# codihuston/eioku

Hardware: AMD Instinct MI355X
Metric: frames/sec (scene+detect+embed) per node (higher is better)
Workload: dtype f16

## Files before the change

### eioku_amd/csrc/yolo.hip

```cpp
#include <algorithm>
#include <array>
#include <memory>
#include <string>
#include <vector>

#include "convnet.h"
#include "yolo_ops.h"

#include <cstdlib>

using namespace eioku;

namespace {

constexpr int kRegMax = 16;

struct Buf {
  int level;
  int ch;
  DevBuf<__half> ptr;
};

enum OpKind { kConv, kPool, kUp };

struct Op {
  OpKind kind;
  int conv = -1;
  int in_buf, in_off, in_ch;
  int out_buf, out_off;
  int res_buf = -1, res_off = 0;
  int act = kActSiLU;
  int f32_out = -1;
  bool pose = false;
  bool chain_next = false;
  bool sole_consumer = false;
  int up_consumer = -1;
  int up_from = -1;
};

}

struct eioku_yolo {
  int ch[5], depth[4], nc, nk = 0;
  ConvStack convs;
  std::vector<Buf> bufs;
  std::vector<Op> ops;
  int in_buf = -1;
  int head_src[3];
  int cur_n = 0, cur_h = 0, cur_w = 0;
  DevBuf<float> head[9];
  DevBuf<float> kpts;
  DevBuf<unsigned long long> clsmax[3];
  DevBuf<int32_t> lvl;
  DevBuf<int32_t> flat;
  int32_t* pass_host = nullptr;
  hipEvent_t pass_event = nullptr;
  bool pass_pending = false;
  long long pass_seen[2] = {0, 0};
  int deep_idx[3][2] = {{-1, -1}, {-1, -1}, {-1, -1}};
  DevBuf<Cand> cands;
  DevBuf<int32_t> counts;
  DevBuf<Det> dets;
  DevBuf<char> lb_tables;
  unsigned long long lb_key = 0;
  void* lb_key_ptr = nullptr;
  __half* lb_out = nullptr;
  double conv_flops_last = 0;
};

namespace {

int add_buf(eioku_yolo* y, int level, int ch) {
  y->bufs.push_back(Buf{level, ch, {}});
  return (int)y->bufs.size() - 1;
}

int add_conv_w(eioku_yolo* y, const std::string& name, int cout, int cin, int k, int s) {
  return y->convs.add({name, cout, cin, k, s});
}

void add_conv(eioku_yolo* y, const std::string& name, int cin, int cout, int k, int s, int in_buf, int in_off,
              int out_buf, int out_off, int res_buf = -1, int res_off = 0, int act = kActSiLU, int f32_out = -1) {
  Op op;
  op.kind = kConv;
  op.conv = add_conv_w(y, name, cout, cin, k, s);
  op.in_buf = in_buf;
  op.in_off = in_off;
  op.in_ch = cin;
  op.out_buf = out_buf;
  op.out_off = out_off;
  op.res_buf = res_buf;
  op.res_off = res_off;
  op.act = act;
  op.f32_out = f32_out;
  y->ops.push_back(op);
}

void add_c2f(eioku_yolo* y, const std::string& p, int level, int c1, int c2, int n, bool shortcut, int in_buf,
             int in_off, int out_buf, int out_off) {
  const int c = c2 / 2;
  const int cat = add_buf(y, level, (2 + n) * c);
  const int tmp = add_buf(y, level, c);
  add_conv(y, p + ".cv1.conv", c1, 2 * c, 1, 1, in_buf, in_off, cat, 0);
  for (int i = 0; i < n; ++i) {
    const std::string m = p + ".m." + std::to_string(i);
    add_conv(y, m + ".cv1.conv", c, c, 3, 1, cat, (1 + i) * c, tmp, 0);
    add_conv(y, m + ".cv2.conv", c, c, 3, 1, tmp, 0, cat, (2 + i) * c, shortcut ? cat : -1, (1 + i) * c);
  }
// ... 110 lines not shown
    if (c.kind == kConv && y->convs.layers[c.conv].k == 1 && c.in_off == 0 && c.in_ch >= up.in_ch && up.in_ch % 32 == 0) {
      up.up_consumer = consumer;
      c.up_from = (int)i;
    }
  }
  for (size_t i = 0; i + 1 < y->ops.size(); ++i) {
    Op& op = y->ops[i];
    if (op.kind != kConv || op.f32_out >= 0 || op.out_buf == y->in_buf) continue;
    int readers = 0;
    for (size_t j = 0; j < y->ops.size(); ++j)
      readers += (y->ops[j].in_buf == op.out_buf) + (y->ops[j].res_buf == op.out_buf);
    const Op& nx = y->ops[i + 1];
    int writers = 0;
    for (const Op& o : y->ops) writers += (o.f32_out < 0 && o.out_buf == op.out_buf);
    op.sole_consumer = readers == 1 && writers == 1 && nx.in_buf == op.out_buf && nx.res_buf != op.out_buf &&
                       y->bufs[op.out_buf].ch == y->convs.layers[op.conv].cout;
    bool priv = nx.in_buf == op.out_buf && nx.in_off == op.out_off && y->bufs[op.out_buf].ch == y->convs.layers[op.conv].cout;
    for (size_t j = 0; j < y->ops.size() && priv; ++j) {
      const Op& o = y->ops[j];
      if (o.res_buf == op.out_buf) priv = false;
      if (o.in_buf == op.out_buf) {
        const Op* pv = j > 0 ? &y->ops[j - 1] : nullptr;
        priv = priv && pv && pv->kind == kConv && pv->f32_out < 0 && pv->out_buf == op.out_buf && pv->out_off == o.in_off;
      }
    }
    op.chain_next = priv;
  }
}

int level_dim(int x, int level) {
  for (int i = 0; i < level; ++i) x = conv_out_dim(x, 3, 2);
  return x;
}

int prepare(eioku_yolo* y, int n, int h, int w) {
  EIOKU_REQUIRE(h % 32 == 0 && w % 32 == 0, "network input %dx%d must be a multiple of 32", h, w);
  for (const auto& b : y->bufs) {
    const long long px = (long long)n * level_dim(h, b.level) * level_dim(w, b.level);
    EIOKU_REQUIRE(px * b.ch < (1ll << 31) && px < (1ll << 24) * 16,
                  "batch of %d frames at %dx%d: an activation tensor of %lld x %d channels exceeds one launch's 32-bit "
                  "offsets -- split the batch", n, h, w, px, b.ch);
  }
  for (auto& b : y->bufs) EIOKU_TRY(grow_synced(b.ptr, (size_t)n * level_dim(h, b.level) * level_dim(w, b.level) * b.ch));
  size_t A = 0;
  for (int l = 0; l < 3; ++l) {
    const size_t px = (size_t)n * level_dim(h, 3 + l) * level_dim(w, 3 + l);
    A += px;
    EIOKU_TRY(grow_synced(y->head[l], px * 4 * kRegMax));
    EIOKU_TRY(grow_synced(y->head[3 + l], px * y->nc));
    EIOKU_TRY(grow_synced(y->clsmax[l], px));
    if (y->nk > 0) EIOKU_TRY(grow_synced(y->head[6 + l], px * y->nk));
  }
  EIOKU_TRY(grow_synced(y->cands, A + (A + 3) / 4));
  EIOKU_TRY(grow_synced(y->counts, (size_t)n * 2));
  EIOKU_TRY(grow_synced(y->lvl, A + (size_t)n * 3));
  EIOKU_TRY(grow_synced(y->flat, 10 * A + 16));
  y->cur_n = n;
  y->cur_h = h;
  y->cur_w = w;
  return EIOKU_OK;
}

__global__ void k_pass_record(const int32_t* counts, int n, int total, int32_t* out) {
  __shared__ int s;
  if (threadIdx.x == 0) s = 0;
  __syncthreads();
  int v = 0;
  for (int i = threadIdx.x; i < n; i += blockDim.x) v += counts[i];
  atomicAdd(&s, v);
  __syncthreads();
  if (threadIdx.x == 0) {
    out[0] = s;
    out[1] = 0;
    out[2] = 0;
    out[3] = total;
  }
}

int record_pass_rate(eioku_yolo* y, int n, int A, hipStream_t stream) {
  int32_t* dev = y->flat + (size_t)10 * n * A + 8;
  hipLaunchKernelGGL(k_pass_record, dim3(1), dim3(256), 0, stream, y->counts.p, n, n * A, dev);
  EIOKU_HIP_CHECK(hipMemcpyAsync(y->pass_host, dev, 4 * sizeof(int32_t), hipMemcpyDeviceToHost, stream));
  EIOKU_HIP_CHECK(hipEventRecord(y->pass_event, stream));
  y->pass_pending = true;
  return EIOKU_OK;
}

int run_ops(eioku_yolo* y, int n, int h, int w, hipStream_t stream, const FusedInput* fused, double* flops_out,
            bool clsmax = false, bool lazybox = false, bool lazydeep = false, bool kpts = false) {
  static const bool up_off = env_off("EIOKU_UP_FUSE");
  double flops = 0;
  bool skip_next = false;
  int pool_skip = 0, front_skip = 0;
  for (const Op& op : y->ops) {
    if (front_skip > 0) {
      --front_skip;
      continue;
    }
    if (skip_next) {
      skip_next = false;
      continue;
    }
    if (op.pose && !kpts) continue;
    const Buf& ib = y->bufs[op.in_buf];
    const int H = level_dim(h, ib.level), W = level_dim(w, ib.level);
    Slice in{ib.ptr, ib.ch, op.in_off};
    int rc = EIOKU_OK;
// ... 299 lines not shown
      EIOKU_HIP_CHECK(hipMemcpyAsync((void*)p.xalpha, xalpha, (size_t)p.new_w * 4, hipMemcpyHostToDevice, stream));
      EIOKU_HIP_CHECK(hipMemcpyAsync((void*)p.ybeta, ybeta, (size_t)p.new_h * 4, hipMemcpyHostToDevice, stream));
      EIOKU_HIP_CHECK(hipStreamSynchronize(stream));
      y->lb_key = key;
      y->lb_key_ptr = t;
    }
  }
  const uint8_t* d_bgr = bgr;
  if (mem == EIOKU_MEM_HOST) {
    uint8_t* s = (uint8_t*)scratch(kSlotIn, (size_t)n * h * w * 3);
    if (!s) return EIOKU_ENOMEM;
    EIOKU_HIP_CHECK(hipMemcpyAsync(s, bgr, (size_t)n * h * w * 3, hipMemcpyHostToDevice, stream));
    d_bgr = s;
  }
  int step = 1, off = 0;
  if (p.mode == 1 && p.new_w > 1 && p.new_h > 1) {
    const int k = xofs[1] - xofs[0];
    bool decim = k >= 2 && yofs[1] - yofs[0] == k && xofs[0] == yofs[0] && xofs[0] >= 0 &&
                 (long long)k * (p.new_w - 1) + xofs[0] <= w - 2 && (long long)k * (p.new_h - 1) + yofs[0] < h;
    for (int i = 0; decim && i < p.new_w; ++i) decim = xofs[i] == k * i + xofs[0] && xalpha[2 * i] == 2048 && xalpha[2 * i + 1] == 0;
    for (int j = 0; decim && j < p.new_h; ++j) decim = yofs[j] == k * j + yofs[0] && ybeta[2 * j] == 2048 && ybeta[2 * j + 1] == 0;
    if (decim) {
      step = k;
      off = xofs[0];
    }
  }
  FusedInput fi{d_bgr, p.src_h, p.src_w, p.new_h, p.new_w, p.top, p.left, step > 1 ? 0 : p.mode, step, off};
  const Op& op0 = y->ops.front();
  static const bool no_fuse = env_off("EIOKU_STEM_FUSE");
  const bool fuse = !no_fuse && op0.kind == kConv && op0.in_buf == y->in_buf && op0.res_buf < 0 && op0.f32_out < 0 &&
                    fused_input_ok(y->convs.w[op0.conv], fi, Slice{}, nullptr);
  if (!fuse) {
    rc = letterbox_forward(d_bgr, n, p, y->bufs[y->in_buf].ptr, stream);
    if (rc) return rc;
  }
  bool cm = true;
  for (const Op& op : y->ops)
    if (op.kind == kConv && op.f32_out >= 3 && op.f32_out < 6) cm = cm && conv_clsmax_ok(y->convs.w[op.conv], op.act);
  static const bool lazy_off = env_off("EIOKU_LAZY_BOX");
  bool lazy = cm && !lazy_off;
  LazyBox lbx{};
  for (const Op& op : y->ops)
    if (op.kind == kConv && op.f32_out >= 0 && op.f32_out < 3) {
      const ConvWeights& cw = y->convs.w[op.conv];
      lazy = lazy && cw.ks == 1 && cw.ntiles == 1 && cw.nf == 4 && cw.cout == 64 && cw.cin % 32 == 0 && op.act == kActNone &&
             op.res_buf < 0 && (lbx.in_cs == 0 || (lbx.in_cs == y->bufs[op.in_buf].ch && lbx.nchunks == cw.nchunks));
      lbx.in[op.f32_out] = y->bufs[op.in_buf].ptr + op.in_off;
      lbx.wgt[op.f32_out] = reinterpret_cast<const uint4*>(cw.d_w.p);
      lbx.bias[op.f32_out] = cw.d_b;
      lbx.in_cs = y->bufs[op.in_buf].ch;
      lbx.nchunks = cw.nchunks;
    }
  static const float deep_frac = (float)env_num("EIOKU_LAZY_DEEP_FRAC", 0.03);
  bool deep = lazy && deep_frac > 0.f;
  int Hq[3], Wq[3], Aq = 0;
  for (int l = 0; l < 3; ++l) {
    Hq[l] = level_dim(p.out_h, 3 + l);
    Wq[l] = level_dim(p.out_w, 3 + l);
    Aq += Hq[l] * Wq[l];
  }
  if (deep) {
    if (!y->pass_host) {
      EIOKU_HIP_CHECK(hipHostMalloc((void**)&y->pass_host, 4 * sizeof(int32_t), hipHostMallocDefault));
      EIOKU_HIP_CHECK(hipEventCreateWithFlags(&y->pass_event, hipEventDisableTiming));
      y->pass_host[0] = y->pass_host[1] = y->pass_host[2] = y->pass_host[3] = 0;
    }
    if (y->pass_pending && hipEventQuery(y->pass_event) == hipSuccess) {
      y->pass_seen[0] = (long long)y->pass_host[0] + y->pass_host[1] + y->pass_host[2];
      y->pass_seen[1] = y->pass_host[3];
      y->pass_pending = false;
    }
    const long long passed = y->pass_seen[0], total = y->pass_seen[1];
    deep = total > 0 && (float)passed <= deep_frac * (float)total;
    int32_t* f = y->flat;
    int32_t* fcnt = f + (size_t)10 * n * Aq;
    size_t off1 = 0, off0 = (size_t)n * Aq;
    for (int l = 0; l < 3 && deep; ++l) {
      const int i0 = y->deep_idx[l][0], i1 = y->deep_idx[l][1];
      if (i0 < 0 || i1 < 0) {
        deep = false;
        break;
      }
      const Op& o0 = y->ops[i0];
      const Op& o1 = y->ops[i1];
      const ConvWeights& w0 = y->convs.w[o0.conv];
      const ConvWeights& w1 = y->convs.w[o1.conv];
      auto ok3 = [](const ConvWeights& w, const Op& o) {
        return w.ks == 3 && w.stride == 1 && w.cout == 64 && w.cin % 32 == 0 && o.act == kActSiLU && o.res_buf < 0 && o.f32_out < 0;
      };
      if (!ok3(w0, o0) || !ok3(w1, o1) || (long long)n * Hq[l] * Wq[l] >= (1ll << 31)) {
        deep = false;
        break;
      }
      lbx.c0[l] = LazyConv3{y->bufs[o0.in_buf].ptr + o0.in_off, y->bufs[o0.in_buf].ch, w0.nchunks,
                            reinterpret_cast<const uint4*>(w0.d_w.p), 16 * w0.nf, w0.d_b,
                            y->bufs[o0.out_buf].ptr + o0.out_off, y->bufs[o0.out_buf].ch};
      lbx.c1[l] = LazyConv3{y->bufs[o1.in_buf].ptr + o1.in_off, y->bufs[o1.in_buf].ch, w1.nchunks,
                            reinterpret_cast<const uint4*>(w1.d_w.p), 16 * w1.nf, w1.d_b,
                            y->bufs[o1.out_buf].ptr + o1.out_off, y->bufs[o1.out_buf].ch};
      lbx.flat1[l] = f + off1;
      lbx.flat0[l] = f + off0;
      off1 += (size_t)n * Hq[l] * Wq[l];
      off0 += (size_t)9 * n * Hq[l] * Wq[l];
    }
    lbx.fcnt = fcnt;
    lbx.deep = deep;
  }
  rc = run_network(y, n, p.out_h, p.out_w, stream, fuse ? &fi : nullptr, cm, lazy, deep, kpts_out != nullptr);
  if (rc) return rc;

  int Hl[3], Wl[3], A = 0;
  for (int l = 0; l < 3; ++l) {
    Hl[l] = level_dim(p.out_h, 3 + l);
    Wl[l] = level_dim(p.out_w, 3 + l);
    A += Hl[l] * Wl[l];
  }
  rc = grow_synced(y->dets, (size_t)n * max_det);
  if (rc) return rc;
  EIOKU_HIP_CHECK(hipMemsetAsync(y->counts, 0, (size_t)n * 2 * sizeof(int32_t), stream));
  const float* box[3] = {y->head[0], y->head[1], y->head[2]};
  const float* cls[3] = {y->head[3], y->head[4], y->head[5]};
  const unsigned long long* cmw[3] = {y->clsmax[0], y->clsmax[1], y->clsmax[2]};
  if (lazy) {
    int32_t* lvl_counts = y->lvl + (size_t)n * A;
    EIOKU_HIP_CHECK(hipMemsetAsync(lvl_counts, 0, (size_t)n * 3 * sizeof(int32_t), stream));
    if (lbx.deep) EIOKU_HIP_CHECK(hipMemsetAsync(lbx.fcnt, 0, 6 * sizeof(int32_t), stream));
    float* boxw[3] = {y->head[0], y->head[1], y->head[2]};
    rc = decode_lazy_forward(boxw, cmw, lbx, n, Hl, Wl, y->nc, conf, y->cands, y->counts, y->lvl, lvl_counts, A, stream);
    if (rc == EIOKU_OK && y->pass_host) rc = record_pass_rate(y, n, A, stream);
  } else {
    rc = decode_forward(box, cm ? nullptr : cls, n, Hl, Wl, y->nc, conf, y->cands, y->counts, A, stream, cm ? cmw : nullptr);
  }
  if (rc) return rc;
  ScaleParams sp;
  sp.gain = gain;
  sp.pad_x = (float)lb_geom[7];
  sp.pad_y = (float)lb_geom[8];
  sp.src_w = (float)w;
  sp.src_h = (float)h;
  rc = nms_forward(y->cands, y->counts, n, A, iou, max_det, 7680.0f, sp, y->dets, y->counts + n, stream);
  if (rc) return rc;
  const hipMemcpyKind kind = mem == EIOKU_MEM_HOST ? hipMemcpyDeviceToHost : hipMemcpyDeviceToDevice;
  if (kpts_out) {
    const float* kp[3] = {y->head[6], y->head[7], y->head[8]};
    const ScaleParams kps{gain, (float)(((double)p.out_w - (double)w * (double)gain) / 2), (float)(((double)p.out_h - (double)h * (double)gain) / 2),
                          (float)w, (float)h};
    EIOKU_TRY(grow_synced(y->kpts, (size_t)n * max_det * y->nk));
    rc = kpts_decode_forward(kp, y->dets, y->counts + n, n, Hl, Wl, y->nk, max_det, kps, y->kpts, stream);
    if (rc) return rc;
    EIOKU_HIP_CHECK(hipMemcpyAsync(kpts_out, y->kpts, (size_t)n * max_det * y->nk * sizeof(float), kind, stream));
  }
  EIOKU_HIP_CHECK(hipMemcpyAsync(dets_out, y->dets, (size_t)n * max_det * sizeof(Det), kind, stream));
  EIOKU_HIP_CHECK(hipMemcpyAsync(counts_out, y->counts + n, (size_t)n * sizeof(int32_t), kind, stream));
  if (mem == EIOKU_MEM_HOST) EIOKU_HIP_CHECK(hipStreamSynchronize(stream));
  return EIOKU_OK;
}

}

extern "C" {

int eioku_letterbox_f16(const uint8_t* bgr_dev, int n, int h, int w, const int32_t* lb_geom, const int32_t* xofs,
                        const int32_t* yofs, const int16_t* xalpha, const int16_t* ybeta, void* out_nhwc8_dev,
                        void* stream_) {
  EIOKU_REQUIRE_INIT();
  EIOKU_REQUIRE(lb_geom && (n == 0 || (bgr_dev && out_nhwc8_dev)), "NULL argument");
  hipStream_t stream = (hipStream_t)stream_;
  LetterboxPlan p;
  p.src_h = h; p.src_w = w;
  p.new_h = lb_geom[0]; p.new_w = lb_geom[1]; p.top = lb_geom[2]; p.left = lb_geom[3];
  p.out_h = lb_geom[4]; p.out_w = lb_geom[5]; p.mode = lb_geom[6];
  EIOKU_REQUIRE(p.mode >= 0 && p.mode <= 2, "bad letterbox mode %d", p.mode);
  EIOKU_REQUIRE(p.mode != 1 || (xofs && yofs && xalpha && ybeta), "bilinear letterbox needs its tables");
  char* t = (char*)scratch(kSlotWork0, (size_t)(p.new_w + p.new_h) * 8 + 64);
  if (!t) return EIOKU_ENOMEM;
  p.xofs = (const int32_t*)t;
  p.yofs = (const int32_t*)(t + (size_t)p.new_w * 4);
  p.xalpha = (const int16_t*)(t + (size_t)p.new_w * 4 + (size_t)p.new_h * 4);
  p.ybeta = (const int16_t*)(t + (size_t)p.new_w * 8 + (size_t)p.new_h * 4);
  if (p.mode == 1) {
    for (int i = 0; i < p.new_w; ++i) EIOKU_REQUIRE(xofs[i] >= 0 && xofs[i] < w, "xofs[%d]=%d outside the frame", i, xofs[i]);
    EIOKU_HIP_CHECK(hipMemcpyAsync((void*)p.xofs, xofs, (size_t)p.new_w * 4, hipMemcpyHostToDevice, stream));
    EIOKU_HIP_CHECK(hipMemcpyAsync((void*)p.yofs, yofs, (size_t)p.new_h * 4, hipMemcpyHostToDevice, stream));
    EIOKU_HIP_CHECK(hipMemcpyAsync((void*)p.xalpha, xalpha, (size_t)p.new_w * 4, hipMemcpyHostToDevice, stream));
    EIOKU_HIP_CHECK(hipMemcpyAsync((void*)p.ybeta, ybeta, (size_t)p.new_h * 4, hipMemcpyHostToDevice, stream));
  }
  return letterbox_forward(bgr_dev, n, p, (__half*)out_nhwc8_dev, stream);
}

int eioku_yolo_postprocess(const float* const* box_dev, const float* const* cls_dev, int n, const int* hl,
                           const int* wl, int nc, float conf, float iou, int max_det, float gain, int pad_x,
                           int pad_y, int src_w, int src_h, void* dets_dev, int32_t* counts_dev, void* stream_) {
  return eioku_yolo_postprocess_pose(box_dev, cls_dev, nullptr, n, hl, wl, nc, 0, conf, iou, max_det, gain, pad_x, pad_y, 0.f,
                                     0.f, src_w, src_h, dets_dev, counts_dev, nullptr, stream_);
}

int eioku_yolo_postprocess_pose(const float* const* box_dev, const float* const* cls_dev, const float* const* kpt_dev, int n,
                                const int* hl, const int* wl, int nc, int nk, float conf, float iou, int max_det, float gain,
                                int pad_x, int pad_y, float kpad_x, float kpad_y, int src_w, int src_h, void* dets_dev,
                                int32_t* counts_dev, float* kpts_dev, void* stream_) {
  EIOKU_REQUIRE_INIT();
  EIOKU_REQUIRE(!kpts_dev || (kpt_dev && nk > 0 && nk % 3 == 0), "keypoint output without keypoint maps");
  EIOKU_REQUIRE(box_dev && cls_dev && hl && wl && dets_dev && counts_dev, "NULL argument");
  hipStream_t stream = (hipStream_t)stream_;
  if (n == 0) return EIOKU_OK;
  int A = 0;
// ... 19 lines not shown
```

### eioku_amd/csrc/yolo_ops.h

```cpp
#pragma once

#include "conv.h"

namespace eioku {

struct Det {
  float x1, y1, x2, y2;
  float conf;
  int32_t cls;
  int32_t anchor;
  int32_t pad;
};
static_assert(sizeof(Det) == 32, "Det layout is part of the C ABI");

struct Cand {
  float x1, y1, x2, y2;
  float conf;
  int32_t cls;
  int32_t anchor;
  int32_t pad;
};

struct LetterboxPlan {
  int src_h, src_w;
  int new_h, new_w;
  int top, left;
  int out_h, out_w;
  int mode;
  const int32_t* xofs;
  const int32_t* yofs;
  const int16_t* xalpha;
  const int16_t* ybeta;
};
int letterbox_forward(const uint8_t* bgr, int n, const LetterboxPlan& p, __half* out_nhwc8, hipStream_t stream);

int maxpool5_forward(Slice in, Slice out, int N, int H, int W, int C, hipStream_t stream);
int sppf_pools_forward(Slice in, Slice out, int out_step, int N, int H, int W, int C, hipStream_t stream);
int upsample2x_forward(Slice in, Slice out, int N, int H, int W, int C, hipStream_t stream);

int decode_forward(const float* const box[3], const float* const cls[3], int N, const int Hl[3],
                   const int Wl[3], int nc, float conf_thres, Cand* cands, int32_t* counts,
                   int max_cand, hipStream_t stream, const unsigned long long* const clsmax[3] = nullptr);

struct LazyConv3 {
  const __half* in;
  int in_cs, nchunks;
  const uint4* wgt;
  int rows_tile;
  const float* bias;
  __half* out;
  int out_cs;
};
struct LazyBox {
  const __half* in[3];
  const uint4* wgt[3];
  const float* bias[3];
  int in_cs, nchunks;
  bool deep = false;
  LazyConv3 c0[3], c1[3];
  int32_t* flat1[3];
  int32_t* flat0[3];
  int32_t* fcnt;
};
int decode_lazy_forward(float* const box[3], const unsigned long long* const clsmax[3], const LazyBox& lb, int N,
                        const int Hl[3], const int Wl[3], int nc, float conf_thres, Cand* cands, int32_t* counts,
                        int32_t* lvl_list, int32_t* lvl_counts, int max_cand, hipStream_t stream);

struct ScaleParams {
  float gain;
  float pad_x, pad_y;
  float src_w, src_h;
};
int nms_forward(const Cand* cands, const int32_t* counts, int N, int max_cand, float iou_thres,
                int max_det, float max_wh, ScaleParams sp, Det* dets, int32_t* det_counts,
                hipStream_t stream);

int kpts_decode_forward(const float* const kpt[3], const Det* dets, const int32_t* det_counts, int N, const int Hl[3],
                        const int Wl[3], int nk, int max_det, ScaleParams sp, float* out, hipStream_t stream);

}
```

### eioku_amd/csrc/yolo_ops.hip

```cpp
#include "yolo_ops.h"

namespace eioku {

namespace {

struct LbArgs {
  const uint8_t* bgr;
  __half* out;
  int n, src_h, src_w, new_h, new_w, top, left, out_h, out_w, mode;
  const int32_t* xofs;
  const int32_t* yofs;
  const int16_t* xalpha;
  const int16_t* ybeta;
};

__global__ __launch_bounds__(256) void k_letterbox(LbArgs a) {
  const long long total = (long long)a.n * a.out_h * a.out_w;
  long long i = blockIdx.x * 256ll + threadIdx.x;
  if (i >= total) return;
  const int ox = (int)(i % a.out_w);
  const long long t = i / a.out_w;
  const int oy = (int)(t % a.out_h);
  const int n = (int)(t / a.out_h);
  const int y = oy - a.top, x = ox - a.left;
// ... 279 lines not shown
  bool pass = false;
  if (valid) {
    const unsigned long long word = a.cm[lvl][pix];
    const float best = __uint_as_float((unsigned)(word & 0xFFFFFFFFull));
    conf = 1.0f / (1.0f + expf(-best));
    pass = conf > a.conf;
  }
  if (pass) {
    const int pos = atomicAdd(&a.counts[n], 1);
    a.keys[(size_t)n * a.A + pos] =
        ((unsigned long long)__float_as_uint(conf) << 32) | (unsigned long long)(0xFFFFFFFFu - (unsigned)an);
    const int k = atomicAdd(&a.lvl_counts[n * 3 + lvl], 1);
    a.lvl_list[(size_t)n * a.A + a.A0[lvl] + k] = loc;
  }
  if (!a.fcnt) return;
  const int lane = threadIdx.x & 63;
  const int y = loc / W, x = loc - y * W;
  int nb[9], c = 0;
  if (pass) {
#pragma unroll
    for (int dy = -1; dy <= 1; ++dy)
#pragma unroll
      for (int dx = -1; dx <= 1; ++dx)
        if ((unsigned)(y + dy) < (unsigned)H && (unsigned)(x + dx) < (unsigned)W) nb[c++] = (int)pix + dy * W + dx;
  }
  int incl = c;
#pragma unroll
  for (int off = 1; off < 64; off <<= 1) {
    const int v = __shfl_up(incl, off, 64);
    if (lane >= off) incl += v;
  }
  for (int l = 0; l < 3; ++l) {
    const unsigned long long m = __ballot(pass && lvl == l);
    if (m == 0) continue;
    const int leader = __ffsll((long long)m) - 1;
    const int last = 63 - __clzll((long long)m);
    const int before = leader > 0 ? __shfl(incl, leader - 1, 64) : 0;
    const int total0 = __shfl(incl, last, 64) - before;
    int base1 = 0, base0 = 0;
    if (lane == leader) {
      base1 = atomicAdd(&a.fcnt[l], __popcll(m));
      base0 = atomicAdd(&a.fcnt[3 + l], total0);
    }
    base1 = __shfl(base1, leader, 64);
    base0 = __shfl(base0, leader, 64);
    if (pass && lvl == l) {
      a.flat1[l][base1 + __popcll(m & ((1ull << lane) - 1ull))] = (int)pix;
      const int o = base0 + (incl - c) - before;
      for (int i = 0; i < c; ++i) a.flat0[l][o + i] = nb[i];
    }
  }
}

__global__ __launch_bounds__(256) void k_box_gather(DecArgs a) {
  typedef _Float16 half8 __attribute__((ext_vector_type(8)));
  typedef float float4v __attribute__((ext_vector_type(4)));
  const int n = blockIdx.y / 3, lvl = blockIdx.y % 3;
  const int lane = threadIdx.x & 63, wave = threadIdx.x >> 6;
  const int cnt = a.lvl_counts[n * 3 + lvl];
  const int g0 = (blockIdx.x * 4 + wave) * 32;
  if (g0 >= cnt) return;
  const int r = lane & 15, u = lane >> 4;
  const int32_t* list = a.lvl_list + (size_t)n * a.A + a.A0[lvl];
  const size_t img = (size_t)n * a.H[lvl] * a.W[lvl];
  int loc[2];
  const __half* row[2];
#pragma unroll
  for (int m = 0; m < 2; ++m) {
    const int k = g0 + m * 16 + r;
    loc[m] = list[k < cnt ? k : cnt - 1];
    row[m] = a.bin[lvl] + (img + loc[m]) * a.bin_cs + u * 8;
  }
  float4v acc[2][4];
#pragma unroll
  for (int m = 0; m < 2; ++m)
#pragma unroll
    for (int f = 0; f < 4; ++f) acc[m][f] = float4v{0.f, 0.f, 0.f, 0.f};
  const uint4* wl = a.bwgt[lvl] + r * 4 + u;
  float4 biasr[4];
#pragma unroll
  for (int f = 0; f < 4; ++f) biasr[f] = *reinterpret_cast<const float4*>(a.bbias[lvl] + f * 16 + u * 4);
  constexpr int kMaxKc = 4;
  uint4 bfv[kMaxKc][2];
#pragma unroll
  for (int kc = 0; kc < kMaxKc; ++kc)
#pragma unroll
    for (int m = 0; m < 2; ++m) bfv[kc][m] = *reinterpret_cast<const uint4*>(row[m] + (kc < a.bnchunks ? kc : 0) * 32);
#pragma unroll
  for (int kc = 0; kc < kMaxKc; ++kc) {
    if (kc >= a.bnchunks) break;
    half8 bf[2];
#pragma unroll
    for (int m = 0; m < 2; ++m) bf[m] = *reinterpret_cast<const half8*>(&bfv[kc][m]);
#pragma unroll
    for (int f = 0; f < 4; ++f) {
      const uint4 w = wl[(kc * 64 + f * 16) * 4];
      const half8 af = *reinterpret_cast<const half8*>(&w);
#pragma unroll
      for (int m = 0; m < 2; ++m) acc[m][f] = __builtin_amdgcn_mfma_f32_16x16x32_f16(af, bf[m], acc[m][f], 0, 0, 0);
    }
  }
#pragma unroll
  for (int m = 0; m < 2; ++m) {
    if (g0 + m * 16 + r >= cnt) continue;
    float* o = a.box_w[lvl] + (img + loc[m]) * 64;
#pragma unroll
    for (int f = 0; f < 4; ++f) {
      const float4 b = biasr[f];
      *reinterpret_cast<float4v*>(o + f * 16 + u * 4) = acc[m][f] + float4v{b.x, b.y, b.z, b.w};
    }
  }
}

__global__ __launch_bounds__(256) void k_decode_boxes(DecArgs a) {
  const int n = blockIdx.y;
  const int pos = blockIdx.x * 256 + threadIdx.x;
  if (pos >= a.counts[n]) return;
  const unsigned long long key = a.keys[(size_t)n * a.A + pos];
  const int an = (int)(0xFFFFFFFFu - (unsigned)(key & 0xFFFFFFFFull));
  const float conf = __uint_as_float((unsigned)(key >> 32));
  const int lvl = an >= a.A0[2] ? 2 : (an >= a.A0[1] ? 1 : 0);
  const int loc = an - a.A0[lvl];
  const int W = a.W[lvl], H = a.H[lvl];
  const size_t pix = (size_t)n * H * W + loc;
  const int bj = (int)(a.cm[lvl][pix] >> 32);
  const float* bl = a.box[lvl] + pix * 64;
  float side[4];
#pragma unroll
  for (int s = 0; s < 4; ++s) {
    float l[16];
#pragma unroll
    for (int q = 0; q < 4; ++q) {
      const float4 v = *reinterpret_cast<const float4*>(bl + s * 16 + q * 4);
      l[q * 4] = v.x; l[q * 4 + 1] = v.y; l[q * 4 + 2] = v.z; l[q * 4 + 3] = v.w;
    }
    side[s] = dfl_side(l);
  }
  const float stride = (float)(8 << lvl);
  const float ax = (float)(loc % W) + 0.5f, ay = (float)(loc / W) + 0.5f;
  const float bx1 = ax - side[0], by1 = ay - side[1], bx2 = ax + side[2], by2 = ay + side[3];
  const float cx = ((bx1 + bx2) / 2.0f) * stride, cy = ((by1 + by2) / 2.0f) * stride;
  const float w = (bx2 - bx1) * stride, h = (by2 - by1) * stride;
  const float hw = w / 2.0f, hh = h / 2.0f;
  Cand c;
  c.x1 = cx - hw; c.y1 = cy - hh; c.x2 = cx + hw; c.y2 = cy + hh;
  c.conf = conf; c.cls = bj; c.anchor = an; c.pad = 0;
  a.cands[(size_t)n * a.A + an] = c;
}

struct NmsArgs {
  const Cand* cands;
  const unsigned long long* keys;
  const int32_t* counts;
  int A, max_det;
  float iou, max_wh;
  ScaleParams sp;
  Det* dets;
  int32_t* det_counts;
};

__device__ __forceinline__ bool iou_gt(float ax1, float ay1, float ax2, float ay2, float aarea, float bx1,
                                       float by1, float bx2, float by2, float barea, float thr) {
  const float xx1 = fmaxf(ax1, bx1), yy1 = fmaxf(ay1, by1);
  const float xx2 = fminf(ax2, bx2), yy2 = fminf(ay2, by2);
  const float w = fmaxf(0.f, xx2 - xx1), h = fmaxf(0.f, yy2 - yy1);
  const float inter = w * h;
  const float ovr = inter / (aarea + barea - inter);
  return ovr > thr;
}

__global__ __launch_bounds__(256) void k_nms(NmsArgs a) {
  extern __shared__ __attribute__((aligned(16))) unsigned char smem[];
  unsigned long long* key = reinterpret_cast<unsigned long long*>(smem);
  const int n = blockIdx.x, tid = threadIdx.x;
  const int C = min(a.counts[n], a.A);
  int P = 1;
  while (P < C) P <<= 1;
  for (int i = tid; i < P; i += 256) key[i] = i < C ? a.keys[(size_t)n * a.A + i] : 0ull;
  __syncthreads();
  for (int k = 2; k <= P; k <<= 1) {
    for (int j = k >> 1; j > 0; j >>= 1) {
      for (int i = tid; i < P; i += 256) {
        const int l = i ^ j;
        if (l > i) {
          const unsigned long long x = key[i], y = key[l];
          const bool desc = (i & k) == 0;
          if (desc ? (x < y) : (x > y)) {
            key[i] = y;
            key[l] = x;
          }
        }
      }
      __syncthreads();
    }
  }
  if (tid >= 64) return;
  float* kb = reinterpret_cast<float*>(smem + (size_t)(P > 0 ? P : 1) * 8);
  int* kanchor = reinterpret_cast<int*>(kb + 5 * a.max_det);
  const int lane = tid;
  const Cand* cd = a.cands + (size_t)n * a.A;
  int kept = 0;
  for (int base = 0; base < C && kept < a.max_det; base += 64) {
    const int i = base + lane;
    const bool valid = i < C;
    float x1 = 0, y1 = 0, x2 = 0, y2 = 0, area = 0;
    int an = 0;
    if (valid) {
      an = (int)(0xFFFFFFFFu - (unsigned)(key[i] & 0xFFFFFFFFull));
      const Cand c = cd[an];
      const float off = (float)c.cls * a.max_wh;
      x1 = c.x1 + off; y1 = c.y1 + off; x2 = c.x2 + off; y2 = c.y2 + off;
      area = (x2 - x1) * (y2 - y1);
    }
    bool alive = valid;
    for (int k = 0; k < kept; ++k) {
      const float* q = kb + 5 * k;
      if (alive && iou_gt(q[0], q[1], q[2], q[3], q[4], x1, y1, x2, y2, area, a.iou)) alive = false;
    }
    unsigned long long mask = __ballot(alive);
    while (mask != 0 && kept < a.max_det) {
      const int l = __ffsll((long long)mask) - 1;
      const float lx1 = __shfl(x1, l, 64), ly1 = __shfl(y1, l, 64), lx2 = __shfl(x2, l, 64),
                  ly2 = __shfl(y2, l, 64), la = __shfl(area, l, 64);
      const int lan = __shfl(an, l, 64);
      if (lane == 0) {
        float* q = kb + 5 * kept;
        q[0] = lx1; q[1] = ly1; q[2] = lx2; q[3] = ly2; q[4] = la;
        kanchor[kept] = lan;
// ... 214 lines not shown
                        int32_t* lvl_list, int32_t* lvl_counts, int max_cand, hipStream_t stream) {
  if (N == 0) return EIOKU_OK;
  DecArgs a{};
  int A = 0, amax = 0;
  for (int l = 0; l < 3; ++l) {
    a.box[l] = box[l];
    a.box_w[l] = box[l];
    a.cls[l] = nullptr;
    a.cm[l] = clsmax[l];
    a.H[l] = Hl[l];
    a.W[l] = Wl[l];
    a.A0[l] = A;
    A += Hl[l] * Wl[l];
    if (Hl[l] * Wl[l] > amax) amax = Hl[l] * Wl[l];
    a.bin[l] = lb.in[l];
    a.bwgt[l] = lb.wgt[l];
    a.bbias[l] = lb.bias[l];
  }
  EIOKU_REQUIRE(A == max_cand, "candidate capacity %d != anchors %d", max_cand, A);
  a.bin_cs = lb.in_cs;
  EIOKU_REQUIRE(lb.nchunks >= 1 && lb.nchunks <= 4, "box branch input of %d channels: k_box_gather stages at most 128", lb.nchunks * 32);
  a.bnchunks = lb.nchunks;
  a.N = N;
  a.nc = nc;
  a.A = A;
  a.conf = conf_thres;
  a.cands = cands;
  a.keys = reinterpret_cast<unsigned long long*>(cands + (size_t)N * A);
  a.counts = counts;
  a.lvl_list = lvl_list;
  a.lvl_counts = lvl_counts;
  a.fcnt = nullptr;
  if (lb.deep) {
    a.fcnt = lb.fcnt;
    for (int l = 0; l < 3; ++l) {
      a.flat1[l] = lb.flat1[l];
      a.flat0[l] = lb.flat0[l];
    }
  }
  hipLaunchKernelGGL(k_decode_pass, dim3((unsigned)((A + 255) / 256), (unsigned)N), dim3(256), 0, stream, a);
  if (lb.deep) {
    GArgs g0, g1;
    for (int l = 0; l < 3; ++l) {
      g0.l[l] = GConv{lb.c0[l].in, lb.c0[l].wgt, lb.c0[l].bias, lb.c0[l].out, lb.flat0[l], lb.fcnt + 3 + l, Hl[l], Wl[l],
                      lb.c0[l].in_cs, lb.c0[l].out_cs, lb.c0[l].nchunks, lb.c0[l].rows_tile};
      g1.l[l] = GConv{lb.c1[l].in, lb.c1[l].wgt, lb.c1[l].bias, lb.c1[l].out, lb.flat1[l], lb.fcnt + l, Hl[l], Wl[l],
                      lb.c1[l].in_cs, lb.c1[l].out_cs, lb.c1[l].nchunks, lb.c1[l].rows_tile};
    }
    route_hit(route_id(kRouteGather));
    hipLaunchKernelGGL(k_conv3x3_gather, dim3(512, 3), dim3(256), 0, stream, g0);
    route_hit(route_id(kRouteGather));
    hipLaunchKernelGGL(k_conv3x3_gather, dim3(128, 3), dim3(256), 0, stream, g1);
  }
  hipLaunchKernelGGL(k_box_gather, dim3((unsigned)((amax + 127) / 128), (unsigned)(N * 3)), dim3(256), 0, stream, a);
  hipLaunchKernelGGL(k_decode_boxes, dim3((unsigned)((A + 255) / 256), (unsigned)N), dim3(256), 0, stream, a);
  EIOKU_LAUNCH_CHECK();
  return EIOKU_OK;
}

int decode_forward(const float* const box[3], const float* const cls[3], int N, const int Hl[3],
                   const int Wl[3], int nc, float conf_thres, Cand* cands, int32_t* counts, int max_cand,
                   hipStream_t stream, const unsigned long long* const clsmax[3]) {
  if (N == 0) return EIOKU_OK;
  DecArgs a;
  int A = 0;
  for (int l = 0; l < 3; ++l) {
    a.box[l] = box[l];
    a.cls[l] = cls ? cls[l] : nullptr;
    a.cm[l] = clsmax ? clsmax[l] : nullptr;
    a.H[l] = Hl[l];
    a.W[l] = Wl[l];
    a.A0[l] = A;
    A += Hl[l] * Wl[l];
  }
  EIOKU_REQUIRE(A == max_cand, "candidate capacity %d != anchors %d", max_cand, A);
  a.N = N;
  a.nc = nc;
  a.A = A;
  a.conf = conf_thres;
  a.cands = cands;
  a.keys = reinterpret_cast<unsigned long long*>(cands + (size_t)N * A);
  a.counts = counts;
  if (clsmax) hipLaunchKernelGGL(k_decode_cm, dim3(blocks_for((long long)N * A)), dim3(256), 0, stream, a);
  else hipLaunchKernelGGL(k_decode, dim3(blocks_for((long long)N * A * 16)), dim3(256), 0, stream, a);
  EIOKU_LAUNCH_CHECK();
  return EIOKU_OK;
}

int nms_forward(const Cand* cands, const int32_t* counts, int N, int max_cand, float iou_thres, int max_det,
                float max_wh, ScaleParams sp, Det* dets, int32_t* det_counts, hipStream_t stream) {
  if (N == 0) return EIOKU_OK;
  EIOKU_REQUIRE(max_cand <= 16384, "more than 16384 anchors per image (%d) is not supported by the LDS sort", max_cand);
  EIOKU_REQUIRE(max_det > 0 && max_det <= 1024, "max_det %d out of range", max_det);
  int P = 1;
  while (P < max_cand) P <<= 1;
  const size_t lds = (size_t)P * 8 + (size_t)max_det * 6 * 4;
  static size_t lds_attr = 0;
  if (lds > 64 * 1024 && lds > lds_attr) {
    EIOKU_HIP_CHECK(hipFuncSetAttribute(reinterpret_cast<const void*>(k_nms),
                                        hipFuncAttributeMaxDynamicSharedMemorySize, (int)lds));
    lds_attr = lds;
  }
  NmsArgs a;
  a.cands = cands;
  a.keys = reinterpret_cast<const unsigned long long*>(cands + (size_t)N * max_cand);
  a.counts = counts;
  a.A = max_cand;
  a.max_det = max_det;
  a.iou = iou_thres;
  a.max_wh = max_wh;
  a.sp = sp;
  a.dets = dets;
  a.det_counts = det_counts;
  hipLaunchKernelGGL(k_nms, dim3(N), dim3(256), lds, stream, a);
  EIOKU_LAUNCH_CHECK();
  return EIOKU_OK;
}

int kpts_decode_forward(const float* const kpt[3], const Det* dets, const int32_t* det_counts, int N, const int Hl[3],
                        const int Wl[3], int nk, int max_det, ScaleParams sp, float* out, hipStream_t stream) {
  if (N == 0) return EIOKU_OK;
  EIOKU_REQUIRE(nk > 0 && nk % 3 == 0 && max_det > 0, "bad keypoint layout nk=%d max_det=%d", nk, max_det);
  EIOKU_REQUIRE(kpt[0] && kpt[1] && kpt[2] && dets && det_counts && out, "NULL argument");
  KptArgs a;
  for (int l = 0; l < 3; ++l) {
    a.map[l] = kpt[l];
    a.H[l] = Hl[l];
    a.W[l] = Wl[l];
  }
  a.dets = dets;
  a.counts = det_counts;
  a.nk = nk;
  a.max_det = max_det;
  a.sp = sp;
  a.out = out;
  a.total = (long long)N * max_det * (nk / 3);
  hipLaunchKernelGGL(k_kpts_decode, dim3(blocks_for(a.total)), dim3(256), 0, stream, a);
  EIOKU_LAUNCH_CHECK();
  return EIOKU_OK;
}

}
```

Before: 48140.

## Fuse detection tail: box decode into gather, pass-rate into NMS, direct output

Folds the DFL box decode into the box-gather MFMA kernel through an LDS patch, which removes the separate decode launch and the global round trip of box logits. Pass-rate recording moves into the NMS kernel, which writes to mapped host memory, so the record kernel launch goes away. All counters are consolidated into one buffer cleared by a single memset. With device memory, detections are written straight into the caller's output, skipping the device-to-device copies. This adds LDS use in the gather kernel and more coupled code paths.

```diff
diff --git a/eioku_amd/csrc/yolo.hip b/eioku_amd/csrc/yolo.hip
--- a/eioku_amd/csrc/yolo.hip
+++ b/eioku_amd/csrc/yolo.hip
@@ -54,6 +54,7 @@
   DevBuf<int32_t> lvl;
   DevBuf<int32_t> flat;
   int32_t* pass_host = nullptr;
+  int32_t* pass_dev = nullptr;
   hipEvent_t pass_event = nullptr;
   bool pass_pending = false;
   long long pass_seen[2] = {0, 0};
@@ -270,7 +271,7 @@
     if (y->nk > 0) EIOKU_TRY(grow_synced(y->head[6 + l], px * y->nk));
   }
   EIOKU_TRY(grow_synced(y->cands, A + (A + 3) / 4));
-  EIOKU_TRY(grow_synced(y->counts, (size_t)n * 2));
+  EIOKU_TRY(grow_synced(y->counts, (size_t)n * 5 + 8));
   EIOKU_TRY(grow_synced(y->lvl, A + (size_t)n * 3));
   EIOKU_TRY(grow_synced(y->flat, 10 * A + 16));
   y->cur_n = n;
@@ -676,6 +677,7 @@
       lbx.nchunks = cw.nchunks;
     }
   static const float deep_frac = (float)env_num("EIOKU_LAZY_DEEP_FRAC", 0.03);
+  static const bool tail_fuse = !env_off("EIOKU_TAIL_FUSE");
   bool deep = lazy && deep_frac > 0.f;
   int Hq[3], Wq[3], Aq = 0;
   for (int l = 0; l < 3; ++l) {
@@ -686,6 +688,7 @@
   if (deep) {
     if (!y->pass_host) {
       EIOKU_HIP_CHECK(hipHostMalloc((void**)&y->pass_host, 4 * sizeof(int32_t), hipHostMallocDefault));
+      EIOKU_HIP_CHECK(hipHostGetDevicePointer((void**)&y->pass_dev, y->pass_host, 0));
       EIOKU_HIP_CHECK(hipEventCreateWithFlags(&y->pass_event, hipEventDisableTiming));
       y->pass_host[0] = y->pass_host[1] = y->pass_host[2] = y->pass_host[3] = 0;
     }
@@ -697,7 +700,7 @@
     const long long passed = y->pass_seen[0], total = y->pass_seen[1];
     deep = total > 0 && (float)passed <= deep_frac * (float)total;
     int32_t* f = y->flat;
-    int32_t* fcnt = f + (size_t)10 * n * Aq;
+    int32_t* fcnt = tail_fuse ? y->counts + (size_t)5 * n : f + (size_t)10 * n * Aq;
     size_t off1 = 0, off0 = (size_t)n * Aq;
     for (int l = 0; l < 3 && deep; ++l) {
       const int i0 = y->deep_idx[l][0], i1 = y->deep_idx[l][1];
@@ -739,19 +742,31 @@
     Wl[l] = level_dim(p.out_w, 3 + l);
     A += Hl[l] * Wl[l];
   }
-  rc = grow_synced(y->dets, (size_t)n * max_det);
-  if (rc) return rc;
-  EIOKU_HIP_CHECK(hipMemsetAsync(y->counts, 0, (size_t)n * 2 * sizeof(int32_t), stream));
+  const bool direct = tail_fuse && mem == EIOKU_MEM_DEVICE;
+  Det* dets_dev = direct ? (Det*)dets_out : nullptr;
+  int32_t* det_counts = direct ? counts_out : y->counts + n;
+  if (!direct) {
+    rc = grow_synced(y->dets, (size_t)n * max_det);
+    if (rc) return rc;
+    dets_dev = y->dets;
+  }
+  const size_t nzero = tail_fuse && lazy ? (size_t)n * 5 + 6 : (size_t)n * 2;
+  EIOKU_HIP_CHECK(hipMemsetAsync(y->counts, 0, nzero * sizeof(int32_t), stream));
   const float* box[3] = {y->head[0], y->head[1], y->head[2]};
   const float* cls[3] = {y->head[3], y->head[4], y->head[5]};
   const unsigned long long* cmw[3] = {y->clsmax[0], y->clsmax[1], y->clsmax[2]};
+  bool pass_in_nms = false;
   if (lazy) {
-    int32_t* lvl_counts = y->lvl + (size_t)n * A;
-    EIOKU_HIP_CHECK(hipMemsetAsync(lvl_counts, 0, (size_t)n * 3 * sizeof(int32_t), stream));
-    if (lbx.deep) EIOKU_HIP_CHECK(hipMemsetAsync(lbx.fcnt, 0, 6 * sizeof(int32_t), stream));
+    int32_t* lvl_counts = tail_fuse ? y->counts + (size_t)2 * n : y->lvl + (size_t)n * A;
+    if (!tail_fuse) {
+      EIOKU_HIP_CHECK(hipMemsetAsync(lvl_counts, 0, (size_t)n * 3 * sizeof(int32_t), stream));
+      if (lbx.deep) EIOKU_HIP_CHECK(hipMemsetAsync(lbx.fcnt, 0, 6 * sizeof(int32_t), stream));
+    }
+    lbx.fuse_decode = tail_fuse;
     float* boxw[3] = {y->head[0], y->head[1], y->head[2]};
     rc = decode_lazy_forward(boxw, cmw, lbx, n, Hl, Wl, y->nc, conf, y->cands, y->counts, y->lvl, lvl_counts, A, stream);
-    if (rc == EIOKU_OK && y->pass_host) rc = record_pass_rate(y, n, A, stream);
+    pass_in_nms = tail_fuse && y->pass_host;
+    if (rc == EIOKU_OK && y->pass_host && !tail_fuse) rc = record_pass_rate(y, n, A, stream);
   } else {
     rc = decode_forward(box, cm ? nullptr : cls, n, Hl, Wl, y->nc, conf, y->cands, y->counts, A, stream, cm ? cmw : nullptr);
   }
@@ -762,20 +777,27 @@
   sp.pad_y = (float)lb_geom[8];
   sp.src_w = (float)w;
   sp.src_h = (float)h;
-  rc = nms_forward(y->cands, y->counts, n, A, iou, max_det, 7680.0f, sp, y->dets, y->counts + n, stream);
+  rc = nms_forward(y->cands, y->counts, n, A, iou, max_det, 7680.0f, sp, dets_dev, det_counts, stream,
+                   pass_in_nms ? y->pass_dev : nullptr, n * A);
   if (rc) return rc;
+  if (pass_in_nms) {
+    EIOKU_HIP_CHECK(hipEventRecord(y->pass_event, stream));
+    y->pass_pending = true;
+  }
   const hipMemcpyKind kind = mem == EIOKU_MEM_HOST ? hipMemcpyDeviceToHost : hipMemcpyDeviceToDevice;
   if (kpts_out) {
     const float* kp[3] = {y->head[6], y->head[7], y->head[8]};
     const ScaleParams kps{gain, (float)(((double)p.out_w - (double)w * (double)gain) / 2), (float)(((double)p.out_h - (double)h * (double)gain) / 2),
                           (float)w, (float)h};
     EIOKU_TRY(grow_synced(y->kpts, (size_t)n * max_det * y->nk));
-    rc = kpts_decode_forward(kp, y->dets, y->counts + n, n, Hl, Wl, y->nk, max_det, kps, y->kpts, stream);
+    rc = kpts_decode_forward(kp, dets_dev, det_counts, n, Hl, Wl, y->nk, max_det, kps, y->kpts, stream);
     if (rc) return rc;
     EIOKU_HIP_CHECK(hipMemcpyAsync(kpts_out, y->kpts, (size_t)n * max_det * y->nk * sizeof(float), kind, stream));
   }
-  EIOKU_HIP_CHECK(hipMemcpyAsync(dets_out, y->dets, (size_t)n * max_det * sizeof(Det), kind, stream));
-  EIOKU_HIP_CHECK(hipMemcpyAsync(counts_out, y->counts + n, (size_t)n * sizeof(int32_t), kind, stream));
+  if (!direct) {
+    EIOKU_HIP_CHECK(hipMemcpyAsync(dets_out, y->dets, (size_t)n * max_det * sizeof(Det), kind, stream));
+    EIOKU_HIP_CHECK(hipMemcpyAsync(counts_out, y->counts + n, (size_t)n * sizeof(int32_t), kind, stream));
+  }
   if (mem == EIOKU_MEM_HOST) EIOKU_HIP_CHECK(hipStreamSynchronize(stream));
   return EIOKU_OK;
 }
diff --git a/eioku_amd/csrc/yolo_ops.h b/eioku_amd/csrc/yolo_ops.h
--- a/eioku_amd/csrc/yolo_ops.h
+++ b/eioku_amd/csrc/yolo_ops.h
@@ -61,6 +61,7 @@
   int32_t* flat1[3];
   int32_t* flat0[3];
   int32_t* fcnt;
+  bool fuse_decode = false;
 };
 int decode_lazy_forward(float* const box[3], const unsigned long long* const clsmax[3], const LazyBox& lb, int N,
                         const int Hl[3], const int Wl[3], int nc, float conf_thres, Cand* cands, int32_t* counts,
@@ -73,7 +74,7 @@
 };
 int nms_forward(const Cand* cands, const int32_t* counts, int N, int max_cand, float iou_thres,
                 int max_det, float max_wh, ScaleParams sp, Det* dets, int32_t* det_counts,
-                hipStream_t stream);
+                hipStream_t stream, int32_t* pass_out = nullptr, int pass_total = 0);
 
 int kpts_decode_forward(const float* const kpt[3], const Det* dets, const int32_t* det_counts, int N, const int Hl[3],
                         const int Wl[3], int nk, int max_det, ScaleParams sp, float* out, hipStream_t stream);
diff --git a/eioku_amd/csrc/yolo_ops.hip b/eioku_amd/csrc/yolo_ops.hip
--- a/eioku_amd/csrc/yolo_ops.hip
+++ b/eioku_amd/csrc/yolo_ops.hip
@@ -355,9 +355,13 @@
   }
 }
 
+constexpr int kBoxRow = 68;
+
+template <bool kDecode>
 __global__ __launch_bounds__(256) void k_box_gather(DecArgs a) {
   typedef _Float16 half8 __attribute__((ext_vector_type(8)));
   typedef float float4v __attribute__((ext_vector_type(4)));
+  __shared__ __attribute__((aligned(16))) float patch[kDecode ? 4 * 32 * kBoxRow : 4];
   const int n = blockIdx.y / 3, lvl = blockIdx.y % 3;
   const int lane = threadIdx.x & 63, wave = threadIdx.x >> 6;
   const int cnt = a.lvl_counts[n * 3 + lvl];
@@ -403,16 +407,62 @@
       for (int m = 0; m < 2; ++m) acc[m][f] = __builtin_amdgcn_mfma_f32_16x16x32_f16(af, bf[m], acc[m][f], 0, 0, 0);
     }
   }
-#pragma unroll
-  for (int m = 0; m < 2; ++m) {
-    if (g0 + m * 16 + r >= cnt) continue;
-    float* o = a.box_w[lvl] + (img + loc[m]) * 64;
+  if (!kDecode) {
+#pragma unroll
+    for (int m = 0; m < 2; ++m) {
+      if (g0 + m * 16 + r >= cnt) continue;
+      float* o = a.box_w[lvl] + (img + loc[m]) * 64;
+#pragma unroll
+      for (int f = 0; f < 4; ++f) {
+        const float4 b = biasr[f];
+        *reinterpret_cast<float4v*>(o + f * 16 + u * 4) = acc[m][f] + float4v{b.x, b.y, b.z, b.w};
+      }
+    }
+    return;
+  }
+  float* pw = patch + wave * 32 * kBoxRow;
+#pragma unroll
+  for (int m = 0; m < 2; ++m)
 #pragma unroll
     for (int f = 0; f < 4; ++f) {
       const float4 b = biasr[f];
-      *reinterpret_cast<float4v*>(o + f * 16 + u * 4) = acc[m][f] + float4v{b.x, b.y, b.z, b.w};
-    }
-  }
+      *reinterpret_cast<float4v*>(pw + (m * 16 + r) * kBoxRow + f * 16 + u * 4) = acc[m][f] + float4v{b.x, b.y, b.z, b.w};
+    }
+  __builtin_amdgcn_fence(__ATOMIC_ACQ_REL, "workgroup");
+  __builtin_amdgcn_wave_barrier();
+  const int ai = lane & 31, hs = lane >> 5;
+  const int k = g0 + ai;
+  const int aloc = a.lvl_list[(size_t)n * a.A + a.A0[lvl] + (k < cnt ? k : cnt - 1)];
+  float sd[2];
+#pragma unroll
+  for (int s = 0; s < 2; ++s) {
+    float l[16];
+#pragma unroll
+    for (int q = 0; q < 4; ++q) {
+      const float4 v = *reinterpret_cast<const float4*>(pw + ai * kBoxRow + (hs * 2 + s) * 16 + q * 4);
+      l[q * 4] = v.x; l[q * 4 + 1] = v.y; l[q * 4 + 2] = v.z; l[q * 4 + 3] = v.w;
+    }
+    sd[s] = dfl_side(l);
+  }
+  const float o0 = __shfl(sd[0], ai + 32, 64), o1 = __shfl(sd[1], ai + 32, 64);
+  if (hs != 0 || k >= cnt) return;
+  const float side[4] = {sd[0], sd[1], o0, o1};
+  const int W = a.W[lvl];
+  const unsigned long long word = a.cm[lvl][img + aloc];
+  const float best = __uint_as_float((unsigned)(word & 0xFFFFFFFFull));
+  const float conf = 1.0f / (1.0f + expf(-best));
+  const int bj = (int)(word >> 32);
+  const int an = a.A0[lvl] + aloc;
+  const float stride = (float)(8 << lvl);
+  const float ax = (float)(aloc % W) + 0.5f, ay = (float)(aloc / W) + 0.5f;
+  const float bx1 = ax - side[0], by1 = ay - side[1], bx2 = ax + side[2], by2 = ay + side[3];
+  const float cx = ((bx1 + bx2) / 2.0f) * stride, cy = ((by1 + by2) / 2.0f) * stride;
+  const float w = (bx2 - bx1) * stride, h = (by2 - by1) * stride;
+  const float hw = w / 2.0f, hh = h / 2.0f;
+  Cand c;
+  c.x1 = cx - hw; c.y1 = cy - hh; c.x2 = cx + hw; c.y2 = cy + hh;
+  c.conf = conf; c.cls = bj; c.anchor = an; c.pad = 0;
+  a.cands[(size_t)n * a.A + an] = c;
 }
 
 __global__ __launch_bounds__(256) void k_decode_boxes(DecArgs a) {
@@ -460,6 +510,8 @@
   ScaleParams sp;
   Det* dets;
   int32_t* det_counts;
+  int32_t* pass_out;
+  int pass_total;
 };
 
 __device__ __forceinline__ bool iou_gt(float ax1, float ay1, float ax2, float ay2, float aarea, float bx1,
@@ -477,6 +529,13 @@
   unsigned long long* key = reinterpret_cast<unsigned long long*>(smem);
   const int n = blockIdx.x, tid = threadIdx.x;
   const int C = min(a.counts[n], a.A);
+  if (a.pass_out && n == 0 && tid >= 192) {
+    int v = 0;
+    for (int i = tid - 192; i < (int)gridDim.x; i += 64) v += a.counts[i];
+#pragma unroll
+    for (int off = 32; off > 0; off >>= 1) v += __shfl_xor(v, off, 64);
+    if (tid == 192) *reinterpret_cast<int4*>(a.pass_out) = int4{v, 0, 0, a.pass_total};
+  }
   int P = 1;
   while (P < C) P <<= 1;
   for (int i = tid; i < P; i += 256) key[i] = i < C ? a.keys[(size_t)n * a.A + i] : 0ull;
@@ -797,8 +856,13 @@
     route_hit(route_id(kRouteGather));
     hipLaunchKernelGGL(k_conv3x3_gather, dim3(128, 3), dim3(256), 0, stream, g1);
   }
-  hipLaunchKernelGGL(k_box_gather, dim3((unsigned)((amax + 127) / 128), (unsigned)(N * 3)), dim3(256), 0, stream, a);
-  hipLaunchKernelGGL(k_decode_boxes, dim3((unsigned)((A + 255) / 256), (unsigned)N), dim3(256), 0, stream, a);
+  const dim3 bgrid((unsigned)((amax + 127) / 128), (unsigned)(N * 3));
+  if (lb.fuse_decode) {
+    hipLaunchKernelGGL(k_box_gather<true>, bgrid, dim3(256), 0, stream, a);
+  } else {
+    hipLaunchKernelGGL(k_box_gather<false>, bgrid, dim3(256), 0, stream, a);
+    hipLaunchKernelGGL(k_decode_boxes, dim3((unsigned)((A + 255) / 256), (unsigned)N), dim3(256), 0, stream, a);
+  }
   EIOKU_LAUNCH_CHECK();
   return EIOKU_OK;
 }
@@ -833,7 +897,8 @@
 }
 
 int nms_forward(const Cand* cands, const int32_t* counts, int N, int max_cand, float iou_thres, int max_det,
-                float max_wh, ScaleParams sp, Det* dets, int32_t* det_counts, hipStream_t stream) {
+                float max_wh, ScaleParams sp, Det* dets, int32_t* det_counts, hipStream_t stream, int32_t* pass_out,
+                int pass_total) {
   if (N == 0) return EIOKU_OK;
   EIOKU_REQUIRE(max_cand <= 16384, "more than 16384 anchors per image (%d) is not supported by the LDS sort", max_cand);
   EIOKU_REQUIRE(max_det > 0 && max_det <= 1024, "max_det %d out of range", max_det);
@@ -857,6 +922,8 @@
   a.sp = sp;
   a.dets = dets;
   a.det_counts = det_counts;
+  a.pass_out = pass_out;
+  a.pass_total = pass_total;
   hipLaunchKernelGGL(k_nms, dim3(N), dim3(256), lds, stream, a);
   EIOKU_LAUNCH_CHECK();
   return EIOKU_OK;
```

Result: no change. 48260 (median of 4 runs) (+0.2%).
